# chriscoey/Hypatia.jl

Measured on AMD Instinct MI355X. Metric: IPM iterations/sec (+ ms per KKT solve): dense n=5000, PosSemidefTri side 200 (Float64, QRCholDense + CombinedStepper), higher is better.
Workload: dtype f64

## Files before the change

hypatia.jl_amd/csrc/dense.hip:

```cpp
#include <malloc.h>
#include "tds_small.hpp"
#include "hyp_internal.hpp"

#include <fcntl.h>
#include <sys/file.h>
#include <sys/stat.h>
#include <unistd.h>

namespace hyp {

void gemm(Ctx& c, bool transa, GemmArgs a) { HYP_CHECK(gemm_f64_launch(c.stream, transa, a, &c.gemm_scratch)); }

void potrf_diag_launch(hipStream_t st, bool factor, bool invert, int batch, int nblocks, double* A, long lda, long strideA, int n, int k0,
                       double* dinv, long strideD, int* info, int own_cu_lds = 0);
int potrf_diag_own_cu_lds();
void potrf_panel_solve_launch(hipStream_t st, int batch, double* A, long lda, long strideA, int k0, int mcols);
void potrf_diag_mfma_launch(hipStream_t st, int batch, double* A, long lda, long strideA, int n, int k0, int* info, int own_cu_lds,
                            double* tinv = nullptr, long tinv_stride = 0, bool prev_update = false);
bool potrf_tinv_on();
bool potrf_diag_prev_ok();
int potrf_diag_mfma_own_cu_lds();
void potrf_panel_mfma_launch(hipStream_t st, int batch, double* A, long lda, long strideA, int k0, int mcols, int coff = 0,
                             const double* tinv = nullptr, long tinv_stride = 0);

// ... 786 lines not shown
      for (int g = 0; g < 4; ++g) {
        rA[g] = Ys[(rowA + 4 * g) * 16 + li];
        rB[g] = Ys[(rowB + 4 * g) * 16 + li];
      }
      tdr_product<LOWER>(top, nb, wv, Xs, rA, rB);
#pragma unroll
      for (int g = 0; g < 4; ++g) {
        Rs[(rowA + 4 * g) * 16 + li] = rA[g];
        Rs[(rowB + 4 * g) * 16 + li] = rB[g];
      }
      __syncthreads();
      tdr_product<LOWER>(dop, nb, wv, Rs, xA, xB);
    }
    __syncthreads();
#pragma unroll
    for (int g = 0; g < 4; ++g) {
      Xs[(rowA + 4 * g) * 16 + li] = xA[g];
      Xs[(rowB + 4 * g) * 16 + li] = xB[g];
    }
    __syncthreads();
    for (int e = tid; e < NB * 16; e += 256) {
      const int k = e & (NB - 1), c = e >> 7;
      if (k < nb && c0 + c < nrhs) X[(long)(c0 + c) * ldx + k] = Xs[k * 16 + c];
    }
    __syncthreads();
  }
}

void trsm_upper_left_fwd_batched(Ctx& c, int n, int nrhs, const double* U, long ldu, long strideU, const double* dinv, long strideD,
                                 double* X, long ldx, long strideX, int batch) {
  if (n <= 0 || nrhs <= 0 || batch <= 0) return;
  const int nblk = (n + NB - 1) / NB;
  const int refine = std::max(1, trsm_refine_steps());
  for (int kb = 0; kb < nblk; ++kb) {
    const int k0 = kb * NB, nb = std::min(NB, n - k0), m = n - k0 - nb;
    hipLaunchKernelGGL(trsm_diag_refined_fwd_batched_kernel, dim3((nrhs + 16 * TDR_CH - 1) / (16 * TDR_CH), batch), dim3(256), 0, c.stream, U + (long)k0 * ldu + k0, ldu,
                       strideU, dinv + (long)kb * DINV_BLK, strideD, nb, X + k0, ldx, strideX, nrhs, refine);
    HYP_CHECK(hipGetLastError());
    if (m > 0) {
      GemmArgs u{};
      u.M = m; u.N = nrhs; u.K = nb; u.A = U + (long)(k0 + nb) * ldu + k0; u.lda = ldu; u.strideA = strideU;
      u.B = X + k0; u.ldb = ldx; u.strideB = strideX; u.C = X + k0 + nb; u.ldc = ldx; u.strideC = strideX;
      u.alpha = -1; u.beta = 1; u.batch = batch;
      gemm(c, true, u);
    }
  }
}

__global__ void place_dinv_kernel(const double* __restrict__ dinv, long strideD, double* __restrict__ Uinv, long ldi, long strideI,
                                  int n) {
  const int b = blockIdx.z;
  const int l = blockIdx.y;
  const int i = blockIdx.x * blockDim.x + threadIdx.x;
  if (i >= n || l >= n) return;
  double v = 0.0;
  if (i / NB == l / NB) v = dinv[(long)b * strideD + (long)(l / NB) * DINV_BLK + (long)(l % NB) * NB + (i % NB)];
  Uinv[(long)b * strideI + (long)l * ldi + i] = v;
}

void trtri_upper_batched(Ctx& c, int n, const double* U, long ldu, long strideU, const double* dinv, long strideD, double* Uinv,
                         long ldi, long strideI, int batch, DBuf* ws_override) {
  if (n <= 0 || batch <= 0) return;
  hipLaunchKernelGGL(place_dinv_kernel, dim3((n + 127) / 128, n, batch), dim3(128), 0, c.stream, dinv, strideD, Uinv, ldi, strideI, n);
  HYP_CHECK(hipGetLastError());
  const int nblk = (n + NB - 1) / NB;
  if (nblk == 1) return;
  DBuf& ws = ws_override ? *ws_override : c.work_tri;
  ws.ensure((size_t)batch * n * NB * sizeof(double));
  for (int jb = 1; jb < nblk; ++jb) {
    const int j0 = jb * NB, nb = std::min(NB, n - j0);
    GemmArgs t{};
    t.M = j0; t.N = nb; t.K = nb; t.A = U + (long)j0 * ldu; t.lda = ldu; t.strideA = strideU;
    t.B = dinv + (long)jb * DINV_BLK; t.ldb = NB; t.strideB = strideD;
    t.C = ws.d(); t.ldc = n; t.strideC = (long)n * NB; t.alpha = 1; t.beta = 0; t.krange = KR_LE_N; t.batch = batch;
    gemm(c, false, t);
    GemmArgs u{};
    u.M = j0; u.N = nb; u.K = j0; u.A = Uinv; u.lda = ldi; u.strideA = strideI;
    u.B = ws.d(); u.ldb = n; u.strideB = (long)n * NB;
    u.C = Uinv + (long)j0 * ldi; u.ldc = ldi; u.strideC = strideI; u.alpha = -1; u.beta = 0; u.krange = KR_GE_M; u.batch = batch;
    gemm(c, false, u);
  }
}

__global__ __launch_bounds__(256) void coldot_kernel(int m, int ncols, int mode, const double* __restrict__ M, long ld,
                                                     const double* __restrict__ v, const double* base, double alpha, double* out) {
  const int j = blockIdx.x * 4 + (threadIdx.x >> 6);
  if (j >= ncols) return;
  const int lane = threadIdx.x & 63;
  int i0 = 0, i1 = m;
  if (mode == 1) i1 = min(j + 1, m);
  else if (mode == 2) i0 = min(j, m);
  const double* a = M + (long)j * ld;
  double s0 = 0.0, s1 = 0.0, s2 = 0.0, s3 = 0.0;
  int i = i0 + lane;
  for (; i + 192 < i1; i += 256) {
    const double a0 = a[i], a1 = a[i + 64], a2 = a[i + 128], a3 = a[i + 192];
    s0 += a0 * v[i];
    s1 += a1 * v[i + 64];
    s2 += a2 * v[i + 128];
    s3 += a3 * v[i + 192];
  }
  for (; i < i1; i += 64) s0 += a[i] * v[i];
  double s = (s0 + s1) + (s2 + s3);
#pragma unroll
  for (int off = 32; off > 0; off >>= 1) s += __shfl_down(s, off);
  if (lane == 0) out[j] = (base ? base[j] : 0.0) + alpha * s;
}

__global__ __launch_bounds__(256) void coldot_batched_kernel(int m, int ncols, int mode, const double* __restrict__ M, long ld,
                                                             const double* __restrict__ v, const double* base, double alpha, double* out) {
  const int j = blockIdx.x * 4 + (threadIdx.x >> 6);
  if (j >= ncols) return;
  const int lane = threadIdx.x & 63;
  int i0 = 0, i1 = m;
  if (mode == 1) i1 = min(j + 1, m);
  else if (mode == 2) i0 = min(j, m);
  const double* a = M + (long)j * ld;
  const int ilast = max(i1 - 1, 0);
  double av[16], vv[16];
#pragma unroll
  for (int k = 0; k < 16; ++k) {
    const int i = min(i0 + lane + 64 * k, ilast);
    av[k] = a[i];
    vv[k] = v[i];
  }
  const double b = base ? base[j] : 0.0;
  double s0 = 0.0, s1 = 0.0, s2 = 0.0, s3 = 0.0;
#pragma unroll
  for (int g = 0; g < 4; ++g) {
    const int i = i0 + lane + 256 * g;
    if (i + 192 < i1) {
      s0 += av[4 * g] * vv[4 * g];
      s1 += av[4 * g + 1] * vv[4 * g + 1];
      s2 += av[4 * g + 2] * vv[4 * g + 2];
      s3 += av[4 * g + 3] * vv[4 * g + 3];
    } else {
#pragma unroll
      for (int t = 0; t < 3; ++t)
        if (i + 64 * t < i1) s0 += av[4 * g + t] * vv[4 * g + t];
    }
  }
  double s = (s0 + s1) + (s2 + s3);
#pragma unroll
  for (int off = 32; off > 0; off >>= 1) s += __shfl_down(s, off);
  if (lane == 0) out[j] = b + alpha * s;
}

bool coldot_batched_on() {
  static const bool on = [] { const char* e = getenv("HYP_COLDOT_BATCH"); return !(e && atoi(e) == 0); }();
  return on;
}

static void coldot(Ctx& c, int m, int ncols, int mode, const double* M, long ld, const double* v, const double* base, double alpha,
                   double* out) {
  if (ncols <= 0) return;
  if (m <= 1024 && coldot_batched_on())
    hipLaunchKernelGGL(coldot_batched_kernel, dim3((ncols + 3) / 4), dim3(256), 0, c.stream, m, ncols, mode, M, ld, v, base, alpha, out);
  else
    hipLaunchKernelGGL(coldot_kernel, dim3((ncols + 3) / 4), dim3(256), 0, c.stream, m, ncols, mode, M, ld, v, base, alpha, out);
}

void coldot_single(Ctx& c, int m, int ncols, int mode, const double* M, long ld, const double* v, const double* base, double alpha, double* out) {
  coldot(c, m, ncols, mode, M, ld, v, base, alpha, out);
}

__global__ __launch_bounds__(256) void plan_probe_kernel(int phase, int n, int sb, const double* __restrict__ Binv, const double* __restrict__ U, long ldu,
                                                         double* __restrict__ t, unsigned long long* __restrict__ out) {
  const int J = blockIdx.x * 4 + (threadIdx.x >> 6);
  if (J >= n) return;
  const int lane = threadIdx.x & 63;
  const int b = J / sb, j = J - b * sb, r0 = b * sb;
  const double* col = phase == 0 ? Binv + (size_t)b * sb * sb + (size_t)j * sb : U + (size_t)(r0 + j) * ldu + r0;
  double s0 = 0.0, s1 = 0.0;
  for (int i = lane; i <= j; i += 64) {
    const double a = col[i];
    const double v0 = phase == 0 ? 1.0 : t[r0 + i];
    const double v1 = phase == 0 ? ((i & 1) ? -1.0 : 1.0) : t[n + r0 + i];
    s0 = fma(a, v0, s0);
    s1 = fma(a, v1, s1);
  }
#pragma unroll
  for (int off = 32; off > 0; off >>= 1) {
    s0 += __shfl_down(s0, off);
    s1 += __shfl_down(s1, off);
  }
  if (lane != 0) return;
  if (phase == 0) {
    t[J] = s0;
    t[n + J] = s1;
  } else {
    const double e0 = fabs(1.0 - s0), e1 = fabs(((j & 1) ? -1.0 : 1.0) - s1);
    double m = e0 > e1 ? e0 : e1;
    if (!(e0 == e0) || !(e1 == e1)) m = __longlong_as_double(0x7ff8000000000000LL);
    atomicMax(out, (unsigned long long)__double_as_longlong(m));
  }
}

void TriSolvePlan::measure_quality(Ctx& c, const double* U, long ldu) {
  probe_ws.ensure((size_t)(2 * n + 2) * sizeof(double));
  double* t = probe_ws.d();
  unsigned long long* out = reinterpret_cast<unsigned long long*>(t + 2 * n);
  c.zero(out, sizeof(unsigned long long));
  const dim3 grid((n + 3) / 4), blk(256);
  hipLaunchKernelGGL(plan_probe_kernel, grid, blk, 0, c.stream, 0, n, sb, Binv.d(), U, ldu, t, out);
  hipLaunchKernelGGL(plan_probe_kernel, grid, blk, 0, c.stream, 1, n, sb, Binv.d(), U, ldu, t, out);
  HYP_CHECK(hipGetLastError());
  c.d2h(c.h_pinned + 200, out, sizeof(double));
  c.sync();
  rho = c.h_pinned[200];
}

void TriSolvePlan::build(Ctx& c, int n_, const double* U, long ldu, const double* dinv) {
  n = 0;
  sb = c.trsv_plan_sb(n_);
  static const int refine_env = [] { const char* e = getenv("HYP_TRSV_REFINE"); return e ? atoi(e) : -1; }();
  refine_req = refine_env >= 0 ? refine_env : 2;
  refine = refine_req;
  rho = -1.0;
  if (sb <= 0 || n_ <= 0) return;
  const int nsb = (n_ + sb - 1) / sb;
  const size_t blk = (size_t)sb * sb;
  Binv.ensure(nsb * blk * sizeof(double));
  BinvT.ensure(nsb * blk * sizeof(double));
  UT.ensure((size_t)n_ * n_ * sizeof(double));
  work.ensure((size_t)2 * sb * sizeof(double));
  const int nfull = n_ / sb, last = n_ - nfull * sb;
  const long strideU = (long)sb * (ldu + 1), strideD = (long)(sb / NB) * DINV_BLK;
  const bool split = (nfull > 0 && last > 0);
  hipEvent_t e0 = c.aux_event(0), e1 = c.aux_event(1);
  if (split) {
    work2.ensure((size_t)last * NB * sizeof(double));
    HYP_CHECK(hipEventRecord(e0, c.stream));
    HYP_CHECK(hipStreamWaitEvent(c.stream2, e0, 0));
    {
      StreamSwap on_helper(c);
      dev_transpose(c, n_, n_, U, ldu, UT.d(), n_, 1, 0, 0);
      trtri_upper_batched(c, last, U + (long)nfull * strideU, ldu, 0, dinv + (long)nfull * strideD, 0, Binv.d() + nfull * blk, sb, 0, 1, &work2);
      dev_transpose(c, last, last, Binv.d() + nfull * blk, sb, BinvT.d() + nfull * blk, sb, 1, 0, 0);
      HYP_CHECK(hipEventRecord(e1, c.stream));
    }
  }
  if (nfull > 0) trtri_upper_batched(c, sb, U, ldu, strideU, dinv, strideD, Binv.d(), sb, (long)blk, nfull);
  if (!split && last > 0) {
    trtri_upper_batched(c, last, U + (long)nfull * strideU, ldu, 0, dinv + (long)nfull * strideD, 0, Binv.d() + nfull * blk, sb, 0, 1);
    dev_transpose(c, last, last, Binv.d() + nfull * blk, sb, BinvT.d() + nfull * blk, sb, 1, 0, 0);
  }
  if (nfull > 0) dev_transpose(c, sb, sb, Binv.d(), sb, BinvT.d(), sb, nfull, (long)blk, (long)blk);
  if (!split) dev_transpose(c, n_, n_, U, ldu, UT.d(), n_, 1, 0, 0);
  if (split) HYP_CHECK(hipStreamWaitEvent(c.stream, e1, 0));
  n = n_;
  static const int adapt_sel = [] { const char* e = getenv("HYP_TRSV_ADAPT"); return e ? atoi(e) : 3; }();
  const bool adapt = adapt_sel == 1 || (adapt_sel == 2 && owner_class == 0) || (adapt_sel == 3 && owner_class == 1);
  static const double adapt_tol = [] { const char* e = getenv("HYP_TRSV_ADAPT_TOL"); return e ? atof(e) : 1e-10; }();
  ++c.plan_builds;
  if (adapt && refine_req >= 2) {
    measure_quality(c, U, ldu);
    static const bool dbg = [] { const char* e = getenv("HYP_TRSV_ADAPT_DBG"); return e && e[0] == '1'; }();
    if (dbg) fprintf(stderr, "[solve plan] n = %d, super-blocks of %d: rho = %.3e\n", n, sb, rho);
    if (rho == rho && rho <= adapt_tol) { refine = 1; ++c.plan_builds_one_step; }
  }
  ol_prepare(c, ldu);
}

void TriSolvePlan::solve(Ctx& c, const double* U, long ldu, bool trans, double* x) {
  if (ol_usable(c, ldu, 1)) { ol_sweep(c, U, trans ? 0 : 1, x, 0, nullptr, 1); return; }
  const int nsb = (n + sb - 1) / sb;
  const size_t blk = (size_t)sb * sb;
  double* t = work.d();
  double* e = work.d() + sb;
  for (int s = 0; s < nsb; ++s) {
    const int b = trans ? s : nsb - 1 - s;
    const int r0 = b * sb, m = std::min(sb, n - r0);
    double* xb = x + r0;
    const double* Dm = trans ? U + (long)r0 * ldu + r0 : UT.d() + (long)r0 * n + r0;
    const long ldd = trans ? ldu : n;
    const double* Bm = (trans ? Binv.d() : BinvT.d()) + b * blk;
    const int mode = trans ? 1 : 2;
    if (refine == 0) {
      coldot(c, m, m, mode, Bm, sb, xb, nullptr, 1.0, t);
      HYP_CHECK(hipMemcpyAsync(xb, t, (size_t)m * sizeof(double), hipMemcpyDeviceToDevice, c.stream));
    } else {
      coldot(c, m, m, mode, Bm, sb, xb, nullptr, 1.0, t);
      for (int it = 0; it < refine; ++it) {
        coldot(c, m, m, mode, Dm, ldd, t, xb, -1.0, e);
        coldot(c, m, m, mode, Bm, sb, e, t, 1.0, it + 1 == refine ? xb : t);
      }
    }
    if (trans) {
      const int rest = n - (r0 + m);
      coldot(c, m, rest, 0, U + (long)(r0 + m) * ldu + r0, ldu, xb, x + r0 + m, -1.0, x + r0 + m);
    } else {
      coldot(c, m, r0, 0, UT.d() + r0, n, xb, x, -1.0, x);
    }
  }
  HYP_CHECK(hipGetLastError());
}

template <int NC>
__global__ __launch_bounds__(256) void coldotn_kernel(int m, int ncols, int mode, const double* __restrict__ M, long ld,
                                                      const double* __restrict__ v, long ldv, const double* base, long ldb, double alpha,
                                                      double* out, long ldo) {
  const int j = blockIdx.x * 4 + (threadIdx.x >> 6);
  if (j >= ncols) return;
  const int lane = threadIdx.x & 63;
  int i0 = 0, i1 = m;
  if (mode == 1) i1 = min(j + 1, m);
  else if (mode == 2) i0 = min(j, m);
  const double* a = M + (long)j * ld;
  const int ilast = max(i1 - 1, 0);
  double av[16];
#pragma unroll
  for (int k = 0; k < 16; ++k) {
    const int i = i0 + lane + 64 * k;
    av[k] = (i < i1) ? a[min(i, ilast)] : 0.0;
  }
  double s[NC];
#pragma unroll
  for (int cc = 0; cc < NC; ++cc) {
    const double* vc = v + (long)cc * ldv;
    double t0 = 0.0, t1 = 0.0;
#pragma unroll
    for (int k = 0; k < 16; k += 2) {
      t0 += av[k] * vc[min(i0 + lane + 64 * k, ilast)];
      t1 += av[k + 1] * vc[min(i0 + lane + 64 * (k + 1), ilast)];
    }
    s[cc] = t0 + t1;
  }
// ... 397 lines not shown
```

hypatia.jl_amd/csrc/gemm_f64.hpp:

```cpp
#pragma once
#include <hip/hip_runtime.h>
#include <stdint.h>

namespace hyp {

typedef double d4_t __attribute__((ext_vector_type(4)));

enum GemmTri : int {
  GEMM_FULL = 0,
  GEMM_UPPER = 1,
  GEMM_UPPER_RECT = 2,
};

enum GemmKRange : int {
  KR_ALL = 0,
  KR_LE_M = 1,
  KR_GE_M = 2,
  KR_LE_N = 3,
  KR_GE_N = 4,
};

struct GemmArgs {
  int M, N, K;
  const double* A; long lda; long strideA;
  const double* B; long ldb; long strideB;
  double* C; long ldc; long strideC;
  double alpha, beta;
  int tri;
  int krange;
  int batch;
  int tiles_m, tiles_n;
  int cm_blk; long cm_stride;
  int tile_hint;
  int epi;
  int tag;
  int hiprio;
  int tri_off;
  int splitk_req;
  int splitk; int kchunk; double* part; long part_ld; long part_stride;
  int vec2;
  const int* tile_map;
  int splitk_base, tail_q, tail_first, tail_chunk;
  int* tile_cnt;
};

struct GemmScratch {
  double* splitk_ws = nullptr;
  size_t splitk_ws_bytes = 0;
  int* tile_map = nullptr;
  int tile_map_T = -1;
  int* tile_cnt = nullptr;
  long tile_cnt_n = 0;
  struct TrapMap { int tiles_m = 0, tiles_n = 0, tri_off = 0; long nblk = 0; int* map = nullptr; unsigned long used = 0; };
  TrapMap trap[16];
  unsigned long trap_clock = 0;
  void release() {
    for (TrapMap& t : trap) { if (t.map) (void)hipFree(t.map); t = TrapMap(); }
    if (splitk_ws) (void)hipFree(splitk_ws);
    if (tile_map) (void)hipFree(tile_map);
    if (tile_cnt) (void)hipFree(tile_cnt);
    splitk_ws = nullptr; splitk_ws_bytes = 0; tile_map = nullptr; tile_map_T = -1; tile_cnt = nullptr; tile_cnt_n = 0;
  }
};

hipError_t gemm_f64_launch(hipStream_t st, bool transa, GemmArgs a, GemmScratch* scratch = nullptr);
hipError_t schur_syrk_cols(hipStream_t st, GemmArgs a, int c0, int c1, GemmScratch* scratch);
hipError_t schur_syrk_edge(hipStream_t st, const GemmArgs& a, int* N0);

}
```

hypatia.jl_amd/csrc/gemm_f64_kernel.hpp:

```cpp
#pragma once
#include "gemm_f64.hpp"
#include <vector>

namespace hyp {

#ifdef HYP_GEMM_PROBE
__device__ unsigned long long gemm_probe_acc[8];
#define GEMM_PROBE_T(x) const unsigned long long x = __builtin_amdgcn_s_memtime()
#else
#define GEMM_PROBE_T(x)
#endif

constexpr int BK = 16, LDS_S = BK + 2;
typedef const volatile double __attribute__((address_space(3))) lds_cv_f64;
constexpr int GEMM_THREADS = 256;

__device__ __forceinline__ void upper_tile_from_linear(int idx, int& tm, int& tn) {
  int t = (int)((sqrt(8.0 * (double)idx + 1.0) - 1.0) * 0.5);
  while ((long)(t + 1) * (t + 2) / 2 <= idx) ++t;
  while ((long)t * (t + 1) / 2 > idx) --t;
  tn = t;
  tm = idx - t * (t + 1) / 2;
}

template <bool TRANSA, int TW, int TAG>
__global__ __launch_bounds__(GEMM_THREADS, 2)
void gemm_f64_kernel(GemmArgs p) {
  constexpr int BM = 32 * TW, BN = 32 * TW;
  constexpr int REPS = 2 * TW;
  constexpr int WT = 16 * TW;
  __shared__ double lds[2][2][BM * LDS_S];

  const int tid = threadIdx.x;
  const int lane = tid & 63;
  const int wave = tid >> 6;
  const int wm = wave & 1, wn = wave >> 1;
  if (p.hiprio) __builtin_amdgcn_s_setprio(3);

  int tm, tn;
  const int bz = blockIdx.y;
  if (p.tile_map) {
    tm = p.tile_map[2 * blockIdx.x];
    tn = p.tile_map[2 * blockIdx.x + 1];
  } else if (p.tri == GEMM_UPPER) {
    upper_tile_from_linear(blockIdx.x, tm, tn);
  } else {
    tm = blockIdx.x % p.tiles_m;
    tn = blockIdx.x / p.tiles_m;
  }
  const int m0 = tm * BM, n0 = tn * BN;
  if (p.tri == GEMM_UPPER_RECT && m0 > n0 + BN - 1 + p.tri_off) return;

  const double* __restrict__ A = p.A + (long)bz * p.strideA;
  const double* __restrict__ B = p.B + (long)bz * p.strideB;
  double* __restrict__ C = p.C + (long)bz * p.strideC;

  int kbeg = 0, kend = p.K;
  if (p.splitk > 1) {
    int z = blockIdx.z, sub = -1;
    if (p.tail_q > 1) {
      if (z >= p.splitk_base) {
        if ((int)blockIdx.x < p.tail_first) return;
        sub = z - p.splitk_base + 1;
        z = p.splitk_base - 1;
      } else if (z == p.splitk_base - 1 && (int)blockIdx.x >= p.tail_first) {
        sub = 0;
      }
    }
    kbeg = z * p.kchunk;
    kend = min(p.K, kbeg + p.kchunk);
    if (sub >= 0) {
      kbeg += sub * p.tail_chunk;
      kend = min(kend, kbeg + p.tail_chunk);
    }
  }
  switch (p.krange) {
    case KR_LE_M: kend = min(p.K, m0 + BM); break;
    case KR_GE_M: kbeg = min(p.K, m0) & ~(BK - 1); break;
    case KR_LE_N: kend = min(p.K, n0 + BN); break;
    case KR_GE_N: kbeg = min(p.K, n0) & ~(BK - 1); break;
    default: break;
  }

  d4_t acc[TW][TW];
#pragma unroll
  for (int i = 0; i < TW; ++i)
#pragma unroll
    for (int j = 0; j < TW; ++j) acc[i][j] = (d4_t){0.0, 0.0, 0.0, 0.0};

  double ra[REPS], rb[REPS];

  const int lk = tid & 15, lr = tid >> 4;
  constexpr int NN_KSTEP = GEMM_THREADS / BM;
  const int nn_r = tid % BM, nn_k = tid / BM;

  typedef double d2_t __attribute__((ext_vector_type(2)));
  constexpr int REPS2 = REPS / 2;
  const bool fast = TRANSA && p.vec2 && (m0 + BM <= p.M) && (n0 + BN <= p.N);
  const int vk = (tid & 7) * 2, vr = tid >> 3;
  const double* __restrict__ fa = A + (long)(m0 + vr) * p.lda + vk;
  const double* __restrict__ fb = B + (long)(n0 + vr) * p.ldb + vk;

  auto load_tiles_fast = [&](int k0) {
#pragma unroll
    for (int rep = 0; rep < REPS2; ++rep) {
      const d2_t ta = *reinterpret_cast<const d2_t*>(fa + (long)(32 * rep) * p.lda + k0);
      const d2_t tb = *reinterpret_cast<const d2_t*>(fb + (long)(32 * rep) * p.ldb + k0);
      ra[2 * rep] = ta.x; ra[2 * rep + 1] = ta.y;
      rb[2 * rep] = tb.x; rb[2 * rep + 1] = tb.y;
    }
  };
  auto store_tiles_fast = [&](int buf) {
    double* As = lds[buf][0];
    double* Bs = lds[buf][1];
#pragma unroll
    for (int rep = 0; rep < REPS2; ++rep) {
      *reinterpret_cast<d2_t*>(As + (vr + 32 * rep) * LDS_S + vk) = (d2_t){ra[2 * rep], ra[2 * rep + 1]};
      *reinterpret_cast<d2_t*>(Bs + (vr + 32 * rep) * LDS_S + vk) = (d2_t){rb[2 * rep], rb[2 * rep + 1]};
    }
  };

  auto load_tiles = [&](int k0) {
    if (fast && k0 + BK <= kend) {
      load_tiles_fast(k0);
      return;
    }

    const int klast = kend - 1;
    if (TRANSA) {
      const int kc = min(k0 + lk, klast);
#pragma unroll
      for (int rep = 0; rep < REPS; ++rep) ra[rep] = A[(long)min(m0 + lr + 16 * rep, p.M - 1) * p.lda + kc];
    } else {
      const int mc = min(m0 + nn_r, p.M - 1);
#pragma unroll
      for (int rep = 0; rep < REPS; ++rep) ra[rep] = A[(long)min(k0 + nn_k + NN_KSTEP * rep, klast) * p.lda + mc];
    }
    {
      const int kc = min(k0 + lk, klast);
#pragma unroll
      for (int rep = 0; rep < REPS; ++rep) rb[rep] = B[(long)min(n0 + lr + 16 * rep, p.N - 1) * p.ldb + kc];
    }
  };

  auto store_tiles = [&](int buf, int k0) {
    if (fast && k0 + BK <= kend) {
      store_tiles_fast(buf);
      return;
    }
    double* As = lds[buf][0];
    double* Bs = lds[buf][1];
    const double kmask = (k0 + lk < kend) ? 1.0 : 0.0;
    if (TRANSA) {
#pragma unroll
      for (int rep = 0; rep < REPS; ++rep) As[(lr + 16 * rep) * LDS_S + lk] = ra[rep] * ((m0 + lr + 16 * rep < p.M) ? kmask : 0.0);
    } else {
      const double mmask = (m0 + nn_r < p.M) ? 1.0 : 0.0;
#pragma unroll
      for (int rep = 0; rep < REPS; ++rep)
        As[nn_r * LDS_S + nn_k + NN_KSTEP * rep] = ra[rep] * ((k0 + nn_k + NN_KSTEP * rep < kend) ? mmask : 0.0);
    }
#pragma unroll
    for (int rep = 0; rep < REPS; ++rep) Bs[(lr + 16 * rep) * LDS_S + lk] = rb[rep] * ((n0 + lr + 16 * rep < p.N) ? kmask : 0.0);
  };

  const int fr = lane & 15, fk = lane >> 4;

  auto compute = [&](int buf) {
    const double* As = lds[buf][0] + (wm * WT + fr) * LDS_S + fk;
    const double* Bs = lds[buf][1] + (wn * WT + fr) * LDS_S + fk;
#pragma unroll
    for (int kk = 0; kk < BK; kk += 4) {
      double af[TW], bf[TW];
#pragma unroll
#ifdef HYP_GEMM_READ2
      for (int i = 0; i < TW; ++i) af[i] = As[i * 16 * LDS_S + kk];
#pragma unroll
      for (int j = 0; j < TW; ++j) bf[j] = Bs[j * 16 * LDS_S + kk];
#else
      for (int i = 0; i < TW; ++i) af[i] = *(lds_cv_f64*)(As + i * 16 * LDS_S + kk);
#pragma unroll
      for (int j = 0; j < TW; ++j) bf[j] = *(lds_cv_f64*)(Bs + j * 16 * LDS_S + kk);
#endif
#pragma unroll
      for (int j = 0; j < TW; ++j)
#pragma unroll
        for (int i = 0; i < TW; ++i)
          acc[j][i] = __builtin_amdgcn_mfma_f64_16x16x4f64(bf[j], af[i], acc[j][i], 0, 0, 0);
    }
  };

  const int nkt = (kend > kbeg) ? (kend - kbeg + BK - 1) / BK : 0;
#ifdef HYP_GEMM_PROBE
  unsigned long long pr_req = 0, pr_mma = 0, pr_sto = 0, pr_bar = 0;
  GEMM_PROBE_T(pr_birth);
#endif
  if (nkt > 0) {
    load_tiles(kbeg);
    store_tiles(0, kbeg);
    __syncthreads();
    for (int t = 0; t < nkt; ++t) {
      const int buf = t & 1;
      GEMM_PROBE_T(c0);
      if (t + 1 < nkt) load_tiles(kbeg + (t + 1) * BK);
      GEMM_PROBE_T(c1);
      compute(buf);
      GEMM_PROBE_T(c2);
      if (t + 1 < nkt) store_tiles(buf ^ 1, kbeg + (t + 1) * BK);
      GEMM_PROBE_T(c3);
      __syncthreads();
#ifdef HYP_GEMM_PROBE
      const unsigned long long c4 = __builtin_amdgcn_s_memtime();
      pr_req += c1 - c0; pr_mma += c2 - c1; pr_sto += c3 - c2; pr_bar += c4 - c3;
#endif
    }
  }
#ifdef HYP_GEMM_PROBE
  if (lane == 0) {
    atomicAdd(&gemm_probe_acc[0], pr_req); atomicAdd(&gemm_probe_acc[1], pr_mma); atomicAdd(&gemm_probe_acc[2], pr_sto);
    atomicAdd(&gemm_probe_acc[3], pr_bar); atomicAdd(&gemm_probe_acc[4], (unsigned long long)nkt); atomicAdd(&gemm_probe_acc[5], 1ull);
    atomicAdd(&gemm_probe_acc[6], __builtin_amdgcn_s_memtime() - pr_birth);
  }
#endif

  const bool upper = (p.tri != GEMM_FULL);
  if (p.splitk > 1) {
    double* __restrict__ W = p.part + ((long)bz * p.splitk + blockIdx.z) * p.part_stride;
    if (TAG == 1 && p.tile_cnt != nullptr) {
#pragma unroll
      for (int j = 0; j < TW; ++j)
#pragma unroll
        for (int r = 0; r < 4; ++r) {
          const int n = n0 + wn * WT + j * 16 + fk + 4 * r;
          if (n >= p.N) continue;
#pragma unroll
          for (int i = 0; i < TW; ++i) {
            const int m = m0 + wm * WT + i * 16 + fr;
            if (m >= p.M || (upper && m > n + p.tri_off)) continue;
            __hip_atomic_store(&W[(long)n * p.part_ld + m], acc[j][i][r], __ATOMIC_RELAXED, __HIP_MEMORY_SCOPE_AGENT);
          }
        }
      asm volatile("s_waitcnt vmcnt(0)" ::: "memory");
      __shared__ int last_in;
      __syncthreads();
      if (tid == 0) {
        const int expect = (p.tail_q > 1 && (int)blockIdx.x >= p.tail_first) ? p.splitk_base - 1 + p.tail_q : p.splitk_base;
        const int old = __hip_atomic_fetch_add(&p.tile_cnt[blockIdx.x], 1, __ATOMIC_RELAXED, __HIP_MEMORY_SCOPE_AGENT);
        last_in = (old == expect - 1) ? 1 : 0;
        if (last_in) __hip_atomic_store(&p.tile_cnt[blockIdx.x], 0, __ATOMIC_RELAXED, __HIP_MEMORY_SCOPE_AGENT);
      }
      __syncthreads();
      if (!last_in) return;
      const int S = p.splitk_base;
      const int S_extra = (p.tail_q > 1 && (int)blockIdx.x >= p.tail_first) ? p.tail_q - 1 : 0;
      const double* __restrict__ P0 = p.part + (long)bz * p.splitk * p.part_stride;
#pragma unroll
      for (int j = 0; j < TW; ++j)
#pragma unroll
        for (int r = 0; r < 4; ++r) {
          const int n = n0 + wn * WT + j * 16 + fk + 4 * r;
          if (n >= p.N) continue;
#pragma unroll
          for (int i = 0; i < TW; ++i) {
            const int m = m0 + wm * WT + i * 16 + fr;
            if (m >= p.M || (upper && m > n + p.tri_off)) continue;
            const long off = (long)n * p.part_ld + m;
            double s = 0.0;
            for (int z = 0; z < S + S_extra; ++z) s += __hip_atomic_load(&P0[(long)z * p.part_stride + off], __ATOMIC_RELAXED, __HIP_MEMORY_SCOPE_AGENT);
            double* cp = C + (long)n * p.ldc + m;
            *cp = p.alpha * s + (p.beta != 0.0 ? p.beta * (*cp) : 0.0);
          }
        }
      return;
    }
#pragma unroll
    for (int j = 0; j < TW; ++j)
#pragma unroll
      for (int r = 0; r < 4; ++r) {
        const int n = n0 + wn * WT + j * 16 + fk + 4 * r;
        if (n >= p.N) continue;
#pragma unroll
        for (int i = 0; i < TW; ++i) {
          const int m = m0 + wm * WT + i * 16 + fr;
          if (m >= p.M || (upper && m > n + p.tri_off)) continue;
          W[(long)n * p.part_ld + m] = acc[j][i][r];
        }
      }
    return;
  }
// ... 206 lines not shown
}
static hipError_t syrk_edge_launch(hipStream_t st, const GemmArgs& a, int N0, int r) {
  static const int cb_env = [] { const char* e = getenv("HYP_SYRK_EDGE_CB"); return e ? atoi(e) : 8; }();
  const int cb = cb_env;
  for (int e0 = 0; e0 < r; e0 += 8) {
    if (cb == 8) hipLaunchKernelGGL((syrk_edge_kernel<8, 8>), dim3((a.N + 7) / 8), dim3(256), 0, st, a.K, a.N, N0, e0, r, a.A, a.lda, a.alpha, a.beta, a.C, a.ldc);
    else hipLaunchKernelGGL((syrk_edge_kernel<4, 8>), dim3((a.N + 3) / 4), dim3(256), 0, st, a.K, a.N, N0, e0, r, a.A, a.lda, a.alpha, a.beta, a.C, a.ldc);
  }
  return hipGetLastError();
}

hipError_t gemm_f64_launch(hipStream_t st, bool transa, GemmArgs a, GemmScratch* gs) {
  if (a.M <= 0 || a.N <= 0 || a.batch <= 0) return hipSuccess;
  if (a.tag == 1 && transa && a.tri == GEMM_UPPER && a.A == a.B && a.lda == a.ldb && a.batch == 1 && a.epi == 0 &&
      a.krange == KR_ALL && a.M == a.N && a.N >= 1024 && a.N % 128 != 0 && a.N % 128 <= 32 && a.K >= 4096) {
    const int r = a.N % 128, N0 = a.N - r;
    GemmArgs m = a;
    m.M = m.N = N0;
    hipError_t e = gemm_f64_launch(st, transa, m, gs);
    if (e != hipSuccess) return e;
    GemmArgs s = a;
    s.tag = 0; s.M = a.N; s.N = r;
    s.B = a.A + (long)N0 * a.lda;
    s.C = a.C + (long)N0 * a.ldc;
    s.tri = GEMM_UPPER_RECT; s.tri_off = N0;
    s.tile_hint = 64; s.splitk_req = 8;
    if (syrk_edge_ok(a)) return syrk_edge_launch(st, a, N0, r);
    return gemm_f64_launch(st, transa, s, gs);
  }
  const long t128 = (long)((a.M + 127) / 128) * ((a.N + 127) / 128) * a.batch;
  const bool small = (a.tile_hint == 64) || (a.tile_hint == 0 && t128 < 192);
  const int BT = small ? 64 : 128;
  a.tiles_m = (a.M + BT - 1) / BT;
  a.tiles_n = (a.N + BT - 1) / BT;
  long nblk;
  const int* trap_map = nullptr;
  static const bool trap_on = [] { const char* e = getenv("HYP_GEMM_TRAP_MAP"); return !(e && atoi(e) == 0); }();
  if (a.tri == GEMM_UPPER) {
    int T = a.tiles_n;
    nblk = (long)T * (T + 1) / 2;
  } else {
    nblk = (long)a.tiles_m * a.tiles_n;
    if (trap_on && gs && a.tag == 1 && transa && a.tri == GEMM_UPPER_RECT && !small && a.batch == 1 && a.epi == 0 && a.krange == KR_ALL && nblk >= 64) {
      long real = 0;
      trap_map = trap_tile_map(*gs, a.tiles_m, a.tiles_n, a.tri_off, &real);
      if (trap_map) nblk = real;
    }
  }
  a.splitk = 1;
  if (gs && a.tag == 1 && !small && a.batch == 1 && a.epi == 0 && a.krange == KR_ALL && a.K >= 4096) {
    const double eps = (trap_map ? (double)nblk * 16384.0 * 4.6e-12 : (double)a.N * a.N * 2.3e-12) / (2.6e-7 * a.K);
    double best = 1e30;
    for (int S = 1; S <= 8; ++S) {
      if (a.K / S < 1024) break;
      double rounds = (double)((nblk * S + 511) / 512);
      static const bool s_plain = [] { const char* e = getenv("HYP_SYRK_S_PLAIN"); return e && atoi(e) == 1; }();
      static const bool tail_sel = [] { const char* e = getenv("HYP_SYRK_TAIL"); return !(e && atoi(e) == 0); }();
      if (!s_plain && tail_sel && transa && (trap_map || a.tri == GEMM_UPPER) && nblk >= 64 && S > 1) {
        const long rem = (nblk * S) % 512;
        const int kc = (((a.K + S - 1) / S) + BK - 1) / BK * BK;
        if (rem > 0 && rem <= nblk) {
          double last = 1.0;
          for (int q = 2; q <= 4; ++q) {
            const double t = (double)((rem * q + 511) / 512) / q;
            if (t < last - 1e-9 && kc / q >= 256) last = t;
          }
          rounds = (double)((nblk * S) / 512) + last;
        }
      }
      const double cost = rounds / S + (S > 1 ? S * eps : 0.0);
      if (cost < best - 1e-9) { best = cost; a.splitk = S; }
    }
    static const int s_env = [] { const char* e = getenv("HYP_SYRK_S"); return e ? atoi(e) : 0; }();
    if (s_env > 0 && a.K / s_env >= 512) a.splitk = s_env;
  }
  static const bool auto_split = [] { const char* e = getenv("HYP_GEMM_AUTOSPLIT"); return !(e && atoi(e) == 0); }();
  static const long split_max = [] { const char* e = getenv("HYP_GEMM_AUTOSPLIT_MAX"); return e ? atol(e) : 256L; }();
  if (auto_split && gs && a.splitk_req <= 1 && a.batch == 1 && a.epi == 0 && a.krange == KR_ALL && a.cm_blk == 0 && a.K >= 2048 &&
      ((a.tag != 1 && nblk < 128) || (small && nblk >= 128 && nblk < split_max))) {
    const int S = (int)std::min<long>(std::min<long>(16, 512 / nblk), a.K / 256);
    if (S > 1) a.splitk_req = S;
  }
  if (gs && a.splitk_req > 1 && a.epi == 0 && a.krange == KR_ALL && a.cm_blk == 0 && a.K / a.splitk_req >= 256) a.splitk = a.splitk_req;
  a.splitk_base = a.splitk; a.tail_q = 1; a.tail_first = 0; a.tail_chunk = 0;
  if (a.splitk > 1) {
    a.kchunk = (((a.K + a.splitk - 1) / a.splitk) + BK - 1) / BK * BK;
    static const bool tail_on = [] { const char* e = getenv("HYP_SYRK_TAIL"); return !(e && atoi(e) == 0); }();
    if (tail_on && gs && a.tag == 1 && transa && (a.tri == GEMM_UPPER || trap_map) && !small && a.batch == 1 && nblk >= 64) {
      const long rem = (nblk * a.splitk) % 512;
      if (rem > 0 && rem <= nblk) {
        int best_q = 1;
        double best = 1.0;
        for (int q = 2; q <= 4; ++q) {
          const double t = (double)((rem * q + 511) / 512) / q;
          if (t < best - 1e-9 && a.kchunk / q >= 256) { best = t; best_q = q; }
        }
        if (best_q > 1) {
          a.tail_q = best_q;
          a.tail_first = (int)(nblk - rem);
          a.tail_chunk = ((a.kchunk + best_q - 1) / best_q + BK - 1) / BK * BK;
          a.splitk = a.splitk_base + best_q - 1;
        }
      }
    }
    a.part_ld = a.M;
    a.part_stride = (long)a.M * a.N;
    const size_t need = (size_t)a.splitk * a.part_stride * sizeof(double) * (size_t)a.batch;
    if (need > gs->splitk_ws_bytes) {
      if (gs->splitk_ws) (void)hipFree(gs->splitk_ws);
      gs->splitk_ws = nullptr; gs->splitk_ws_bytes = 0;
      hipError_t e = hipMalloc((void**)&gs->splitk_ws, need);
      if (e != hipSuccess) return e;
      gs->splitk_ws_bytes = need;
    }
    a.part = gs->splitk_ws;
  }
  a.vec2 = (transa && ((uintptr_t)a.A % 16 == 0) && ((uintptr_t)a.B % 16 == 0) && (a.lda % 2 == 0) && (a.ldb % 2 == 0) &&
            (a.strideA % 2 == 0) && (a.strideB % 2 == 0) && a.krange != KR_GE_M && a.krange != KR_GE_N) ? 1 : 0;
  a.tile_map = nullptr;
  if (gs && a.tag == 1 && a.tri == GEMM_UPPER && !small && a.batch == 1 && nblk >= 64) a.tile_map = upper_tile_map(*gs, a.tiles_n, nblk);
  if (trap_map) a.tile_map = trap_map;
  if (a.tail_q > 1 && !a.tile_map) { a.splitk = a.splitk_base; a.tail_q = 1; }
  dim3 grid((unsigned)nblk, (unsigned)a.batch, (unsigned)a.splitk);
  a.tile_cnt = nullptr;
  static const bool fuse_red = [] { const char* e = getenv("HYP_SYRK_FUSED_REDUCE"); return e && atoi(e) == 1; }();
  if (fuse_red && gs && a.splitk > 1 && a.tag == 1 && transa && !small && a.batch == 1 && a.tile_map) {
    if (gs->tile_cnt_n < nblk) {
      if (gs->tile_cnt) (void)hipFree(gs->tile_cnt);
      gs->tile_cnt = nullptr; gs->tile_cnt_n = 0;
      if (hipMalloc((void**)&gs->tile_cnt, (size_t)nblk * sizeof(int)) == hipSuccess && hipMemset(gs->tile_cnt, 0, (size_t)nblk * sizeof(int)) == hipSuccess)
        gs->tile_cnt_n = nblk;
    }
    if (gs->tile_cnt_n >= nblk) a.tile_cnt = gs->tile_cnt;
  }
  if (a.tag == 1 && transa && !small) {
    hipLaunchKernelGGL((gemm_f64_kernel<true, 4, 1>), grid, dim3(GEMM_THREADS), 0, st, a);
  } else if (transa) {
    if (small) hipLaunchKernelGGL((gemm_f64_kernel<true, 2, 0>), grid, dim3(GEMM_THREADS), 0, st, a);
    else hipLaunchKernelGGL((gemm_f64_kernel<true, 4, 0>), grid, dim3(GEMM_THREADS), 0, st, a);
  } else {
    if (small) hipLaunchKernelGGL((gemm_f64_kernel<false, 2, 0>), grid, dim3(GEMM_THREADS), 0, st, a);
    else hipLaunchKernelGGL((gemm_f64_kernel<false, 4, 0>), grid, dim3(GEMM_THREADS), 0, st, a);
  }
  if (a.splitk > 1 && a.tile_cnt == nullptr)
    hipLaunchKernelGGL(splitk_reduce_kernel, dim3((a.M + 255) / 256, a.N, a.batch), dim3(256), 0, st, a.M, a.N, a.tri != GEMM_FULL ? 1 : 0, a.tri_off,
                       a.splitk_base, a.part, a.part_ld, a.part_stride, a.alpha, a.beta, a.C, a.ldc, a.tail_q - 1, a.tail_first,
                       a.tile_map ? a.tile_map + 2 * nblk : nullptr, trap_map ? a.tiles_m : a.tiles_n, (long)a.splitk * a.part_stride, a.strideC);
  return hipGetLastError();
}

hipError_t schur_syrk_cols(hipStream_t st, GemmArgs a, int c0, int c1, GemmScratch* gs) {
  static const int s_env = [] { const char* e = getenv("HYP_CHOL_SPLIT_S"); return e ? atoi(e) : 0; }();
  if (c0 == 0) {
    GemmArgs l = a;
    l.M = l.N = c1;
    if (s_env > 0) l.splitk_req = s_env;
    return gemm_f64_launch(st, true, l, gs);
  }
  const int N = a.N;
  int r = N % 128, N0 = N - r;
  if (!(r > 0 && r <= 32 && a.K >= 4096 && syrk_edge_ok(a))) { r = 0; N0 = N; }
  GemmArgs t = a;
  t.M = N0; t.N = N0 - c0;
  t.B = a.A + (long)c0 * a.lda;
  t.C = a.C + (long)c0 * a.ldc;
  t.tri = GEMM_UPPER_RECT; t.tri_off = c0;
  if (t.N > 0) {
    const long tm = (t.M + 127) / 128, tn = (t.N + 127) / 128, tc0 = c0 / 128;
    long real = 0;
    for (long j = 0; j < tn; ++j) real += std::min(tm, tc0 + j + 1);
    int S = 1;
    double best = 1e30;
    const double eps = ((double)t.M * t.N * 4.6e-12) / (2.6e-7 * a.K);
    for (int q = 1; q <= 8; ++q) {
      if (a.K / q < 1024) break;
      const double cost = (double)((real * q + 511) / 512) / q + (q > 1 ? q * eps : 0.0);
      if (cost < best - 1e-9) { best = cost; S = q; }
    }
    if (s_env > 0) S = s_env;
    t.splitk_req = S;
    hipError_t e = gemm_f64_launch(st, true, t, gs);
    if (e != hipSuccess) return e;
  }
  if (r > 0) return syrk_edge_launch(st, a, N0, r);
  return hipSuccess;
}

hipError_t schur_syrk_edge(hipStream_t st, const GemmArgs& a, int* N0) {
  const int r = a.N % 128;
  *N0 = a.N;
  if (!(r > 0 && r <= 32 && a.N >= 1024 && a.K >= 4096 && a.M == a.N && syrk_edge_ok(a))) return hipSuccess;
  *N0 = a.N - r;
  return syrk_edge_launch(st, a, *N0, r);
}

}
```

Baseline: 56.86.

## Invert triangular super-blocks by recursive doubling with two-level batched GEMMs

```diff
diff --git a/hypatia.jl_amd/csrc/dense.hip b/hypatia.jl_amd/csrc/dense.hip
--- a/hypatia.jl_amd/csrc/dense.hip
+++ b/hypatia.jl_amd/csrc/dense.hip
@@ -892,6 +892,60 @@
   }
 }
 
+bool trtri_doubling_on() {
+  static const bool on = [] { const char* e = getenv("HYP_TRTRI_DOUBLING"); return !(e && atoi(e) == 0); }();
+  return on;
+}
+
+static void trtri_upper_doubling(Ctx& c, int m, const double* U, long ldu, long strideU, const double* dinv, long strideD, double* X,
+                                 long ldi, long strideI, int batch, DBuf& ws) {
+  if (m <= 0 || batch <= 0) return;
+  hipLaunchKernelGGL(place_dinv_kernel, dim3((m + 127) / 128, m, batch), dim3(128), 0, c.stream, dinv, strideD, X, ldi, strideI, m);
+  HYP_CHECK(hipGetLastError());
+  size_t need = 0;
+  for (int h = NB; h < m; h *= 2) {
+    const int nreg = m / (2 * h), nc = m - nreg * 2 * h - h;
+    need = std::max(need, (size_t)batch * ((size_t)nreg * h * h + (size_t)h * std::max(nc, 0)));
+  }
+  ws.ensure(need * sizeof(double));
+  for (int h = NB; h < m; h *= 2) {
+    const int nreg = m / (2 * h);
+    const int p = nreg * 2 * h;
+    const int nc = m - p - h;
+    const long hh = (long)h * h, pairU = 2L * h * (ldu + 1), pairX = 2L * h * (ldi + 1);
+    double* Treg = ws.d();
+    double* Tirr = ws.d() + (size_t)batch * nreg * hh;
+    GemmArgs t{}, u{};
+    t.M = h; t.lda = ldu; t.ldb = ldi; t.ldc = h; t.alpha = 1; t.beta = 0; t.krange = KR_LE_N;
+    u.M = h; u.K = h; u.lda = ldi; u.ldb = h; u.ldc = ldi; u.alpha = -1; u.beta = 0; u.krange = KR_GE_M;
+    if (nreg > 0) {
+      GemmArgs t1 = t, u1 = u;
+      t1.N = h; t1.K = h; t1.batch = batch * nreg; t1.batch_in = nreg;
+      t1.A = U + (long)h * ldu; t1.strideA = pairU; t1.strideA2 = strideU;
+      t1.B = X + (long)h * (ldi + 1); t1.strideB = pairX; t1.strideB2 = strideI;
+      t1.C = Treg; t1.strideC = hh; t1.strideC2 = nreg * hh;
+      gemm(c, false, t1);
+      u1.N = h; u1.batch = batch * nreg; u1.batch_in = nreg;
+      u1.A = X; u1.strideA = pairX; u1.strideA2 = strideI;
+      u1.B = Treg; u1.strideB = hh; u1.strideB2 = nreg * hh;
+      u1.C = X + (long)h * ldi; u1.strideC = pairX; u1.strideC2 = strideI;
+      gemm(c, false, u1);
+    }
+    if (nc > 0) {
+      t.N = nc; t.K = nc; t.batch = batch;
+      t.A = U + (long)(p + h) * ldu + p; t.strideA = strideU;
+      t.B = X + (long)(p + h) * (ldi + 1); t.strideB = strideI;
+      t.C = Tirr; t.strideC = (long)h * nc;
+      gemm(c, false, t);
+      u.N = nc; u.batch = batch;
+      u.A = X + (long)p * (ldi + 1); u.strideA = strideI;
+      u.B = Tirr; u.strideB = (long)h * nc;
+      u.C = X + (long)(p + h) * ldi + p; u.strideC = strideI;
+      gemm(c, false, u);
+    }
+  }
+}
+
 __global__ __launch_bounds__(256) void coldot_kernel(int m, int ncols, int mode, const double* __restrict__ M, long ld,
                                                      const double* __restrict__ v, const double* base, double alpha, double* out) {
   const int j = blockIdx.x * 4 + (threadIdx.x >> 6);
@@ -1038,6 +1092,11 @@
   const long strideU = (long)sb * (ldu + 1), strideD = (long)(sb / NB) * DINV_BLK;
   const bool split = (nfull > 0 && last > 0);
   hipEvent_t e0 = c.aux_event(0), e1 = c.aux_event(1);
+  const bool doubling = trtri_doubling_on();
+  auto invert = [&](int m, const double* Ub, long sU, const double* db, long sD, double* Xb, long sX, int batch, DBuf* ws) {
+    if (doubling) trtri_upper_doubling(c, m, Ub, ldu, sU, db, sD, Xb, sb, sX, batch, ws ? *ws : c.work_tri);
+    else trtri_upper_batched(c, m, Ub, ldu, sU, db, sD, Xb, sb, sX, batch, ws);
+  };
   if (split) {
     work2.ensure((size_t)last * NB * sizeof(double));
     HYP_CHECK(hipEventRecord(e0, c.stream));
@@ -1045,14 +1104,14 @@
     {
       StreamSwap on_helper(c);
       dev_transpose(c, n_, n_, U, ldu, UT.d(), n_, 1, 0, 0);
-      trtri_upper_batched(c, last, U + (long)nfull * strideU, ldu, 0, dinv + (long)nfull * strideD, 0, Binv.d() + nfull * blk, sb, 0, 1, &work2);
+      invert(last, U + (long)nfull * strideU, 0, dinv + (long)nfull * strideD, 0, Binv.d() + nfull * blk, 0, 1, &work2);
       dev_transpose(c, last, last, Binv.d() + nfull * blk, sb, BinvT.d() + nfull * blk, sb, 1, 0, 0);
       HYP_CHECK(hipEventRecord(e1, c.stream));
     }
   }
-  if (nfull > 0) trtri_upper_batched(c, sb, U, ldu, strideU, dinv, strideD, Binv.d(), sb, (long)blk, nfull);
+  if (nfull > 0) invert(sb, U, strideU, dinv, strideD, Binv.d(), (long)blk, nfull, nullptr);
   if (!split && last > 0) {
-    trtri_upper_batched(c, last, U + (long)nfull * strideU, ldu, 0, dinv + (long)nfull * strideD, 0, Binv.d() + nfull * blk, sb, 0, 1);
+    invert(last, U + (long)nfull * strideU, 0, dinv + (long)nfull * strideD, 0, Binv.d() + nfull * blk, 0, 1, nullptr);
     dev_transpose(c, last, last, Binv.d() + nfull * blk, sb, BinvT.d() + nfull * blk, sb, 1, 0, 0);
   }
   if (nfull > 0) dev_transpose(c, sb, sb, Binv.d(), sb, BinvT.d(), sb, nfull, (long)blk, (long)blk);
diff --git a/hypatia.jl_amd/csrc/gemm_f64.hpp b/hypatia.jl_amd/csrc/gemm_f64.hpp
--- a/hypatia.jl_amd/csrc/gemm_f64.hpp
+++ b/hypatia.jl_amd/csrc/gemm_f64.hpp
@@ -42,6 +42,7 @@
   const int* tile_map;
   int splitk_base, tail_q, tail_first, tail_chunk;
   int* tile_cnt;
+  int batch_in; long strideA2, strideB2, strideC2;
 };
 
 struct GemmScratch {
diff --git a/hypatia.jl_amd/csrc/gemm_f64_kernel.hpp b/hypatia.jl_amd/csrc/gemm_f64_kernel.hpp
--- a/hypatia.jl_amd/csrc/gemm_f64_kernel.hpp
+++ b/hypatia.jl_amd/csrc/gemm_f64_kernel.hpp
@@ -51,9 +51,16 @@
   const int m0 = tm * BM, n0 = tn * BN;
   if (p.tri == GEMM_UPPER_RECT && m0 > n0 + BN - 1 + p.tri_off) return;
 
-  const double* __restrict__ A = p.A + (long)bz * p.strideA;
-  const double* __restrict__ B = p.B + (long)bz * p.strideB;
-  double* __restrict__ C = p.C + (long)bz * p.strideC;
+  long offA = (long)bz * p.strideA, offB = (long)bz * p.strideB, offC = (long)bz * p.strideC;
+  if (p.batch_in > 0) {
+    const long bo = bz / p.batch_in, bi = bz - bo * p.batch_in;
+    offA = bi * p.strideA + bo * p.strideA2;
+    offB = bi * p.strideB + bo * p.strideB2;
+    offC = bi * p.strideC + bo * p.strideC2;
+  }
+  const double* __restrict__ A = p.A + offA;
+  const double* __restrict__ B = p.B + offB;
+  double* __restrict__ C = p.C + offC;
 
   int kbeg = 0, kend = p.K;
   if (p.splitk > 1) {
@@ -577,6 +584,7 @@
     if (S > 1) a.splitk_req = S;
   }
   if (gs && a.splitk_req > 1 && a.epi == 0 && a.krange == KR_ALL && a.cm_blk == 0 && a.K / a.splitk_req >= 256) a.splitk = a.splitk_req;
+  if (a.batch_in > 0 && (a.splitk > 1 || a.batch % a.batch_in != 0)) return hipErrorInvalidValue;
   a.splitk_base = a.splitk; a.tail_q = 1; a.tail_first = 0; a.tail_chunk = 0;
   if (a.splitk > 1) {
     a.kchunk = (((a.K + a.splitk - 1) / a.splitk) + BK - 1) / BK * BK;
```

Result: no change. 57.59, median of 4 (+1.3%).

## Software-pipeline LDS fragment reads with MFMA in SYRK kernel and skip dead-warp compute

Applied to the files above, without the earlier changes.

```diff
diff --git a/hypatia.jl_amd/csrc/gemm_f64.hpp b/hypatia.jl_amd/csrc/gemm_f64.hpp
--- a/hypatia.jl_amd/csrc/gemm_f64.hpp
+++ b/hypatia.jl_amd/csrc/gemm_f64.hpp
@@ -42,6 +42,7 @@
   const int* tile_map;
   int splitk_base, tail_q, tail_first, tail_chunk;
   int* tile_cnt;
+  int pipe;
 };
 
 struct GemmScratch {
diff --git a/hypatia.jl_amd/csrc/gemm_f64_kernel.hpp b/hypatia.jl_amd/csrc/gemm_f64_kernel.hpp
--- a/hypatia.jl_amd/csrc/gemm_f64_kernel.hpp
+++ b/hypatia.jl_amd/csrc/gemm_f64_kernel.hpp
@@ -195,16 +195,112 @@
   unsigned long long pr_req = 0, pr_mma = 0, pr_sto = 0, pr_bar = 0;
   GEMM_PROBE_T(pr_birth);
 #endif
-  if (nkt > 0) {
-    load_tiles(kbeg);
-    store_tiles(0, kbeg);
+  int t0 = 0;
+  bool dead = false;
+  if constexpr (TRANSA && TW == 4 && TAG == 1) {
+    dead = (p.pipe & 2) && p.tri != GEMM_FULL && (m0 + WT * wm > n0 + WT * wn + WT - 1 + p.tri_off);
+    const int nfull = (kend > kbeg) ? (kend - kbeg) / BK : 0;
+    if ((p.pipe & 1) && fast && nfull > 0) {
+      load_tiles_fast(kbeg);
+      store_tiles_fast(0);
+      __syncthreads();
+      if (dead) {
+        for (int t = 0; t + 1 < nfull; ++t) {
+          GEMM_PROBE_T(c0);
+          load_tiles_fast(kbeg + (t + 1) * BK);
+          GEMM_PROBE_T(c1);
+          store_tiles_fast((t & 1) ^ 1);
+          GEMM_PROBE_T(c2);
+          __syncthreads();
+#ifdef HYP_GEMM_PROBE
+          const unsigned long long c3 = __builtin_amdgcn_s_memtime();
+          pr_req += c1 - c0; pr_sto += c2 - c1; pr_bar += c3 - c2;
+#endif
+        }
+      } else {
+        double a0[TW], b0[TW], a1[TW], b1[TW];
+        auto frag = [&](int buf, int kk, double* af, double* bf) {
+          const double* As = lds[buf][0] + (wm * WT + fr) * LDS_S + fk + kk;
+          const double* Bs = lds[buf][1] + (wn * WT + fr) * LDS_S + fk + kk;
+#pragma unroll
+          for (int i = 0; i < TW; ++i) af[i] = *(lds_cv_f64*)(As + i * 16 * LDS_S);
+#pragma unroll
+          for (int j = 0; j < TW; ++j) bf[j] = *(lds_cv_f64*)(Bs + j * 16 * LDS_S);
+        };
+        auto mma = [&](const double* af, const double* bf) {
+#pragma unroll
+          for (int j = 0; j < TW; ++j)
+#pragma unroll
+            for (int i = 0; i < TW; ++i)
+              acc[j][i] = __builtin_amdgcn_mfma_f64_16x16x4f64(bf[j], af[i], acc[j][i], 0, 0, 0);
+        };
+        auto reads_then_mmas = [] {
+          __builtin_amdgcn_sched_group_barrier(0x100, 2 * TW, 0);
+          __builtin_amdgcn_sched_group_barrier(0x008, TW * TW, 0);
+        };
+        frag(0, 0, a0, b0);
+        for (int t = 0; t + 1 < nfull; ++t) {
+          const int buf = t & 1;
+          GEMM_PROBE_T(c0);
+          load_tiles_fast(kbeg + (t + 1) * BK);
+          GEMM_PROBE_T(c1);
+          __builtin_amdgcn_sched_barrier(0);
+          frag(buf, 4, a1, b1);
+          mma(a0, b0);
+          frag(buf, 8, a0, b0);
+          mma(a1, b1);
+          reads_then_mmas();
+          reads_then_mmas();
+          __builtin_amdgcn_sched_barrier(0);
+          GEMM_PROBE_T(c2);
+          store_tiles_fast(buf ^ 1);
+          GEMM_PROBE_T(c3);
+          __builtin_amdgcn_sched_barrier(0);
+          frag(buf, 12, a1, b1);
+          mma(a0, b0);
+          reads_then_mmas();
+          __builtin_amdgcn_sched_barrier(0);
+          GEMM_PROBE_T(c4);
+          __syncthreads();
+          GEMM_PROBE_T(c5);
+          __builtin_amdgcn_sched_barrier(0);
+          frag(buf ^ 1, 0, a0, b0);
+          mma(a1, b1);
+          reads_then_mmas();
+          __builtin_amdgcn_sched_barrier(0);
+#ifdef HYP_GEMM_PROBE
+          const unsigned long long c6 = __builtin_amdgcn_s_memtime();
+          pr_req += c1 - c0; pr_mma += (c2 - c1) + (c4 - c3) + (c6 - c5); pr_sto += c3 - c2; pr_bar += c5 - c4;
+#endif
+        }
+        {
+          const int buf = (nfull - 1) & 1;
+          GEMM_PROBE_T(c0);
+          frag(buf, 4, a1, b1);
+          mma(a0, b0);
+          frag(buf, 8, a0, b0);
+          mma(a1, b1);
+          frag(buf, 12, a1, b1);
+          mma(a0, b0);
+          mma(a1, b1);
+#ifdef HYP_GEMM_PROBE
+          pr_mma += __builtin_amdgcn_s_memtime() - c0;
+#endif
+        }
+      }
+      t0 = nfull;
+    }
+  }
+  if (t0 < nkt) {
+    load_tiles(kbeg + t0 * BK);
+    store_tiles(t0 & 1, kbeg + t0 * BK);
     __syncthreads();
-    for (int t = 0; t < nkt; ++t) {
+    for (int t = t0; t < nkt; ++t) {
       const int buf = t & 1;
       GEMM_PROBE_T(c0);
       if (t + 1 < nkt) load_tiles(kbeg + (t + 1) * BK);
       GEMM_PROBE_T(c1);
-      compute(buf);
+      if (!dead) compute(buf);
       GEMM_PROBE_T(c2);
       if (t + 1 < nkt) store_tiles(buf ^ 1, kbeg + (t + 1) * BK);
       GEMM_PROBE_T(c3);
@@ -629,6 +725,8 @@
     if (gs->tile_cnt_n >= nblk) a.tile_cnt = gs->tile_cnt;
   }
   if (a.tag == 1 && transa && !small) {
+    static const int pipe = [] { const char* e = getenv("HYP_SYRK_PIPE"); const int v = e ? atoi(e) : 1; return v == 1 ? 3 : v == 2 ? 1 : v == 3 ? 2 : 0; }();
+    a.pipe = pipe;
     hipLaunchKernelGGL((gemm_f64_kernel<true, 4, 1>), grid, dim3(GEMM_THREADS), 0, st, a);
   } else if (transa) {
     if (small) hipLaunchKernelGGL((gemm_f64_kernel<true, 2, 0>), grid, dim3(GEMM_THREADS), 0, st, a);
```

Result: slower. 58.17 before, 57.57 after (-1.0%).
